# sjpollard/video-how-do-your-tokens-merge

Measured on AMD Instinct MI355X. Metric: clips/sec at r=16, VideoMAE-B 16x224x224 (forward with ToMe merge; merge indices bit-exact against the fp32-arithmetic oracle, which the reference's fp32 fixtures pin), higher is better.
Workload: dtype bf16; 1 GPU; VideoMAE-B random-init, synthetic 16x224x224 clips, r=16, bf16 (BASELINE.json configs[1]); r=16, parallelism=dp1: independent replicas, one RCCL all-reduce of [top1, top5, clips], step_launch=eager

## Files before the change

### include/tome_hip.h

```cpp
#ifndef TOME_HIP_H
#define TOME_HIP_H

#include <stddef.h>
#include <stdint.h>

#ifdef __cplusplus
extern "C" {
#endif

typedef void *tome_stream_t;

enum tome_dtype { TOME_F32 = 0, TOME_BF16 = 1, TOME_F16 = 2 };

enum tome_mode { TOME_SUM = 0, TOME_MEAN = 1, TOME_AMAX = 2, TOME_PROD = 3, TOME_AMIN = 4 };

enum tome_status {
    TOME_OK = 0,
    TOME_EINVAL = 1,
    TOME_EWORKSPACE = 2,
    TOME_ELAUNCH = 3
};

#define TOME_ABI_VERSION 11

// ... 59 lines not shown
                 void *x_out, void *y_out, const void *x_out_bias, tome_stream_t stream);

int tome_drop_regrouped_ln(const void *x, int dtype, int64_t B, int64_t F, int64_t P, int64_t C, int64_t r,
                           int has_cls, const int64_t *und_idx, const void *ln_weight, const void *ln_bias, float eps,
                           const void *addend, int addend_grouped, const void *cls_addend, void *x_out, void *y_out,
                           const void *x_out_bias, tome_stream_t stream);

int tome_prop_attention(const void *q, const void *k, const void *v, int dtype, int64_t B, int64_t H, int64_t N,
                        int64_t Nk, int64_t D, const int64_t *q_strides, const int64_t *k_strides,
                        const int64_t *v_strides, const float *log_size, int64_t log_size_stride, int bias_skip,
                        float scale, void *out, const int64_t *out_strides, tome_stream_t stream);

int tome_prop_attention_segments(const void *q, const void *k, const void *v, int dtype, int64_t B, int64_t H,
                                 int64_t N, int64_t Nk, int64_t D, const int64_t *q_strides,
                                 const int64_t *k_strides, const int64_t *v_strides, const float *log_size,
                                 int64_t log_size_stride, float scale, void *out, const int64_t *out_strides,
                                 int64_t nseg, const int64_t *seg_strides, tome_stream_t stream);

int tome_trajectory_mix(const void *q2, const void *k2, const void *val, int dtype, int64_t B, int64_t S, int64_t F,
                        int64_t H, int64_t D, int64_t k_row_stride, int64_t v_row_stride, float scale, void *out,
                        int64_t out_batch_stride, float *tattn, tome_stream_t stream);

int tome_short_attention(const void *q, const void *k, const void *v, int dtype, int64_t B, int64_t H, int64_t N,
                         int64_t D, const int64_t *q_strides, const int64_t *k_strides, const int64_t *v_strides,
                         float scale, void *out, tome_stream_t stream);

int tome_add_layernorm(const void *x, const void *addend, int dtype, int64_t rows, int64_t C,
                       const void *ln_weight, const void *ln_bias, float eps, void *x_out, void *y_out,
                       tome_stream_t stream);

int tome_add_layernorm_skip_first(const void *x, const void *addend, int dtype, int64_t groups, int64_t group_rows,
                                  int64_t C, const void *ln_weight, const void *ln_bias, float eps, void *x_out,
                                  void *y_out, tome_stream_t stream);

int tome_add_layernorm_regrouped(const void *x, const void *addend, int dtype, int64_t B, int64_t F, int64_t P,
                                 int64_t C, const void *ln_weight, const void *ln_bias, float eps, void *x_out,
                                 void *y_out, tome_stream_t stream);

int tome_merge(const void *x, int dtype, int64_t n, int64_t T, int64_t C, int64_t r,
               const int64_t *src_idx, const int64_t *dst_idx, const int64_t *unm_idx,
               int distill_token, int mode, const uint8_t *edge_keep, void *out,
               tome_stream_t stream);

int tome_drop(const void *x, int dtype, int64_t n, int64_t T, int64_t C, int64_t r,
              const int64_t *und_idx, int distill_token, void *out, tome_stream_t stream);

int tome_unmerge(const void *x, int dtype, int64_t n, int64_t T, int64_t C, int64_t r,
                 const int64_t *src_idx, const int64_t *dst_idx, const int64_t *unm_idx, void *out,
                 tome_stream_t stream);

int tome_merge_backward(const void *grad_out, int x_dtype, const void *out_div, const void *in_mul, int size_dtype,
                        int64_t n, int64_t T, int64_t C, int64_t r, const int32_t *row_map, int distill_token,
                        int drop, void *grad_in, tome_stream_t stream);
int tome_merge_backward_regrouped(const void *grad_out, int x_dtype, const void *out_div, const void *in_mul,
                                  int size_dtype, int64_t B, int64_t F, int64_t P, int64_t C, int64_t r, int has_cls,
                                  const int32_t *row_map, int drop, void *grad_in, tome_stream_t stream);

size_t tome_layernorm_backward_workspace_bytes(int64_t rows, int64_t C);
int tome_layernorm_backward(const void *gy, const void *xs, const void *gx_in, int dtype, int64_t groups,
                            int64_t group_rows, int skip_first, int64_t C, const void *weight, float eps, void *gx,
                            void *dweight, void *dbias, void *workspace, tome_stream_t stream);

size_t tome_layernorm_backward_regrouped_workspace_bytes(int64_t B, int64_t F, int64_t P, int64_t C);
int tome_layernorm_backward_regrouped(const void *gy, const void *xs, const void *gx_in, int dtype, int64_t B, int64_t F,
                                      int64_t P, int64_t C, const void *weight, float eps, void *gx, void *dweight,
                                      void *dbias, void *workspace, tome_stream_t stream);
// ... 112 lines not shown
```

### video-how-do-your-tokens-merge_amd/csrc/tome_kernels.hip

```cpp
#include <hip/hip_runtime.h>
#include <stdarg.h>
#include <stdint.h>
#include <stdio.h>
#include <stdlib.h>
#include <string.h>

#include <type_traits>

#include "../../include/tome_hip.h"
#include "tome_common.h"
#include "tome_match.h"
#include "tome_match_filter.h"
#include "tome_ln_rows.h"
#include "tome_merge_slab.h"
#include "tome_merge.h"
#include "tome_merge_ln_amp.h"
#include "tome_ln_fwd.h"
#include "tome_merge_bwd.h"
#include "tome_ln_bwd.h"
#include "tome_merge_ln_bwd.h"
#include "tome_merge_ln_bwd_amp.h"
#include "tome_gelu.h"
#include "tome_gelu_bwd.h"
#include "tome_token_mean.h"
// ... 606 lines not shown
}

extern "C" int tome_merge_wavg_regrouped_ln(const void *x, int x_dtype, const void *size, int size_dtype, int64_t B,
                                            int64_t F, int64_t P, int64_t C, int64_t r, int has_cls,
                                            const int64_t *src_idx, const int64_t *dst_idx,
                                            const int64_t *unm_idx, const uint8_t *edge_keep, const void *ln_weight,
                                            const void *ln_bias, float eps, const void *addend,
                                            int addend_grouped, const void *cls_addend, void *x_out,
                                            void *y_out, void *size_out, void *log_size_out,
                                            const void *x_out_bias, tome_stream_t stream) {
    if (x_out_bias && !aligned16(x_out_bias))
        return fail(TOME_EINVAL, "tome_merge_wavg_regrouped_ln: x_out_bias not 16-byte aligned");
    if (!y_out || !ln_weight || !ln_bias) return fail(TOME_EINVAL, "tome_merge_wavg_regrouped_ln: null buffer");
    if (x_dtype == TOME_F32) return fail(TOME_EINVAL, "tome_merge_wavg_regrouped_ln: 16-bit tokens only");
    if ((addend && !aligned16(addend)) || (cls_addend && !aligned16(cls_addend)))
        return fail(TOME_EINVAL, "tome_merge_wavg_regrouped_ln: addend alignment");
    if (addend_grouped && !addend) return fail(TOME_EINVAL, "tome_merge_wavg_regrouped_ln: addend_grouped without addend");
    LnArgs ln{ln_weight, ln_bias, y_out, eps, addend, 0, TokLayout{0, 0, 0, 0, 1}, nullptr, x_out_bias};
    if (addend_grouped) {
        const int64_t cls = has_cls ? 1 : 0;
        ln.a_own = 1;
        ln.la = TokLayout{cls * C, (cls + P) * C, 0, C, 1};
        ln.cls_addend = cls_addend;
    }
    return merge_wavg_regrouped_impl("tome_merge_wavg_regrouped_ln", x, x_dtype, size, size_dtype, B, F, P, C, r,
                                     has_cls, src_idx, dst_idx, unm_idx, edge_keep, x_out, size_out, log_size_out, &ln, stream);
}

static inline int ln_rows_per_wave(int64_t cpr, int nit) {
    const int64_t R = (nit * WAVE) / cpr;
    return R > FAST_MAXR ? FAST_MAXR : (int)R;
}

template <typename TS, typename TA, typename TY, typename TP>
static int launch_add_ln_rows(const char *who, const void *x, const void *addend, int64_t rows, int64_t C,
                              const void *ln_weight, const void *ln_bias, float eps, int64_t y_group, void *x_out,
                              void *y_out, tome_stream_t stream) {
    const int64_t cpr = C / 8;
    const int R = ln_rows_per_wave(cpr, 3);
    const int64_t waves = (rows + R - 1) / R;
    if ((waves + 3) / 4 > 0x7fffffffLL) return fail(TOME_EINVAL, "%s: too many rows", who);
    hipLaunchKernelGGL((k_add_ln_rows<TS, TA, TY, TP, 3>), dim3((unsigned)((waves + 3) / 4)), dim3(256), 0,
                       (hipStream_t)stream, (const TS *)x, (const TA *)addend, rows, (int)C, R, (int)cpr,
                       (const TP *)ln_weight, (const TP *)ln_bias, eps, (int)y_group, (TS *)x_out, (TY *)y_out);
    return check_launch("k_add_ln_rows");
}

static int add_layernorm_impl(const void *x, const void *addend, int dtype, int64_t rows, int64_t C,
                              const void *ln_weight, const void *ln_bias, float eps, void *x_out, void *y_out,
                              int64_t y_group, tome_stream_t stream) {
    if (!x || !ln_weight || !ln_bias || (addend && !x_out) || !y_out || rows <= 0 || C <= 0)
        return fail(TOME_EINVAL, "tome_add_layernorm: bad shape/pointer");
    if (int rc = not_16bit("tome_add_layernorm", dtype)) return rc;
    if (C % 8 || C / 8 > 2 * WAVE || !aligned16(x) || !aligned16(addend) || (addend && !aligned16(x_out)) ||
        !aligned16(y_out) || !aligned16(ln_weight) || !aligned16(ln_bias))
        return fail(TOME_EINVAL, "tome_add_layernorm: C %% 8 == 0, C <= 1024 and 16-byte aligned buffers required");
    return dispatch_x<false>(dtype, [&](auto tx) {
        using TX = typename decltype(tx)::type;
        return launch_add_ln_rows<TX, TX, TX, TX>("tome_add_layernorm", x, addend, rows, C, ln_weight, ln_bias, eps,
                                                  y_group, x_out, y_out, stream);
    }, [&] { return not_16bit("tome_add_layernorm", dtype); });
}

extern "C" int tome_add_layernorm(const void *x, const void *addend, int dtype, int64_t rows, int64_t C,
                                  const void *ln_weight, const void *ln_bias, float eps, void *x_out, void *y_out,
                                  tome_stream_t stream) {
    return add_layernorm_impl(x, addend, dtype, rows, C, ln_weight, ln_bias, eps, x_out, y_out, 0, stream);
}

extern "C" int tome_add_layernorm_skip_first(const void *x, const void *addend, int dtype, int64_t groups,
                                             int64_t group_rows, int64_t C, const void *ln_weight,
                                             const void *ln_bias, float eps, void *x_out, void *y_out,
                                             tome_stream_t stream) {
    if (groups <= 0 || group_rows < 2 || group_rows > 0x7fffffffLL)
        return fail(TOME_EINVAL, "tome_add_layernorm_skip_first: groups of at least two rows required");
    return add_layernorm_impl(x, addend, dtype, groups * group_rows, C, ln_weight, ln_bias, eps, x_out, y_out, group_rows,
                              stream);
}

extern "C" int tome_add_layernorm_regrouped(const void *x, const void *addend, int dtype, int64_t B, int64_t F, int64_t P,
                                            int64_t C, const void *ln_weight, const void *ln_bias, float eps,
                                            void *x_out, void *y_out, tome_stream_t stream) {
    if (!x || !addend || !x_out || !y_out || !ln_weight || !ln_bias || B <= 0 || F <= 0 || P <= 0 || C <= 0)
        return fail(TOME_EINVAL, "tome_add_layernorm_regrouped: bad shape/pointer");
    if (int rc = not_16bit("tome_add_layernorm_regrouped", dtype)) return rc;
    const int64_t cpr = C / 8;
    if (C % 8 || cpr > 2 * WAVE || !aligned16(x) || !aligned16(addend) || !aligned16(x_out) || !aligned16(y_out) ||
        !aligned16(ln_weight) || !aligned16(ln_bias))
        return fail(TOME_EINVAL, "tome_add_layernorm_regrouped: C %% 8 == 0, C <= 1024 and 16-byte aligned buffers required");
    const int64_t rows = B * (1 + P * F);
    if (rows > 0x7fffffffLL) return fail(TOME_EINVAL, "tome_add_layernorm_regrouped: too many rows");
    const int R = ln_rows_per_wave(cpr, 3);
    if (R < 1) return fail(TOME_EINVAL, "tome_add_layernorm_regrouped: row too wide");
    const int64_t waves = (rows + R - 1) / R;
    const LnArgs ln{ln_weight, ln_bias, y_out, eps, nullptr, 0, TokLayout{0, 0, 0, 0, 1}, nullptr, nullptr};
    const dim3 grid((unsigned)((waves + 3) / 4));
    hipStream_t st = (hipStream_t)stream;
    return dispatch_x<false>(dtype, [&](auto tx) {
        using TX = typename decltype(tx)::type;
        hipLaunchKernelGGL((k_add_ln_regroup<TX, 3>), grid, dim3(256), 0, st, (const TX *)x, (const TX *)addend, (int)B,
// ... 1353 lines not shown
```

### video-how-do-your-tokens-merge_amd/csrc/tome_ln_fwd.h

```cpp
#pragma once
template <typename TS, typename TA, typename TY, typename TP, int NIT>
__global__ __launch_bounds__(256) void k_add_ln_rows(const TS *__restrict__ x, const TA *__restrict__ a, int64_t rows,
                                                     int C, int R, int cpr, const TP *__restrict__ lw,
                                                     const TP *__restrict__ lb, float eps, int y_group,
                                                     TS *__restrict__ xout, TY *__restrict__ y) {
    const int lane = threadIdx.x & 63;
    const int64_t w = (int64_t)blockIdx.x * (blockDim.x >> 6) + __builtin_amdgcn_readfirstlane(threadIdx.x >> 6);
    const int64_t row0 = w * R;
    if (row0 >= rows) return;
    const int nrow = (int)((rows - row0) < R ? (rows - row0) : R);
    const int total = nrow * cpr;
    const bool add = a != nullptr;
    const TS *xs = x + row0 * C;
    const TA *as = a + row0 * C;
    Slot<TS> raw[NIT] = {};
    Slot<TA> rawa[NIT] = {};
    int rowof[NIT];
#pragma unroll
    for (int it = 0; it < NIT; ++it) {
        const int q = it * WAVE + lane;
        rowof[it] = q < total ? slab_row(cpr, it, lane) : -1;
        if (q < total) {
            raw[it] = ld_slot<TS>(xs, q);
            if (add) rawa[it] = ld_slot<TA>(as, q);
        }
    }
    const LnParams<TP, NIT> prm = ln_params<TP, NIT>(lw, lb, rowof, cpr, lane);
    if (add) {
#pragma unroll
        for (int it = 0; it < NIT; ++it) {
            if (rowof[it] < 0) continue;
            raw[it] = slot_add<TS, TA>(raw[it], rawa[it]);
            st_slot<TS>(xout + row0 * C, it * WAVE + lane, raw[it]);
        }
    }
    ln_rows<TS, TP, TY, NIT>(raw, rowof, nrow, cpr, C, eps, prm, lane,
                             [&](int rr, int cc, const Slot<TY> &yv) __attribute__((always_inline)) {
                                 int64_t yrow = row0 + rr;
                                 if (y_group > 0) {
                                     const int64_t gb = yrow / y_group;
                                     if (yrow - gb * y_group == 0) return;
                                     yrow -= gb + 1;
                                 }
                                 st_slot<TY>(y + yrow * C, cc, yv);
                             });
}

template <typename TX, int NIT>
__global__ __launch_bounds__(256) void k_add_ln_regroup(const TX *__restrict__ x, const TX *__restrict__ a, int B, int F,
                                                        int P, int C, int R, int cpr, LnArgs ln,
                                                        TX *__restrict__ xout) {
    const int lane = threadIdx.x & 63;
    const int64_t w = (int64_t)blockIdx.x * (blockDim.x >> 6) + __builtin_amdgcn_readfirstlane(threadIdx.x >> 6);
    const int N = 1 + P * F;
    const int64_t rows = (int64_t)B * N;
    const int64_t row0 = w * R;
    if (row0 >= rows) return;
// ... 52 lines not shown
```

### video-how-do-your-tokens-merge_amd/tome/_abi.py

```python
from __future__ import annotations

import ctypes
import os
from typing import Optional

import torch

_PKG = os.path.dirname(os.path.dirname(os.path.abspath(__file__)))
LIB_PATH = os.environ.get("TOME_HIP_LIB", os.path.join(_PKG, "lib", "libtome_hip.so"))

i64, i32, vp, sz, f32 = ctypes.c_int64, ctypes.c_int, ctypes.c_void_p, ctypes.c_size_t, ctypes.c_float
SIGNATURES = {
    "tome_abi_version": (i32, [], False),
    "tome_last_error": (ctypes.c_char_p, [], False),
    "tome_effective_r": (i64, [i64, i64, i32, i32], False),
    "tome_match_workspace_bytes": (sz, [i64, i64, i64], False),
    "tome_match": (i32, [vp, i32, i64, i64, i64, i64, i64, i64, i32, i32, vp, vp, vp, vp, vp, vp, sz, vp], False),
    "tome_match_keys": (i32, [vp, i32, i64, i64, i64, i64, i64, i64, i64, i64, i64, i64, i32, i32, vp, vp, vp, vp, vp,
                             vp, sz, vp], False),
    "tome_match_scores": (i32, [vp, i64, i64, i64, i32, i32, vp, vp, vp, vp, vp, vp, sz, vp], False),
    "tome_edge_keep": (i32, [vp, vp, i64, i64, i64, f32, vp, vp], False),
    "tome_merge_wavg": (i32, [vp, i32, vp, i32, i64, i64, i64, i64, vp, vp, vp, i32, vp, vp, vp, vp, vp], False),
    "tome_merge_wavg_ln": (i32, [vp, i32, vp, i32, i64, i64, i64, i64, vp, vp, vp, i32, vp, vp, vp, f32, vp, vp, vp, vp,
                                vp, vp, vp], False),
# ... 34 lines not shown
    "tome_prop_attention_backward": (i32, [vp, vp, vp, vp, vp, i32, i64, i64, i64, i64, i64, vp, vp, vp, vp, vp, vp,
                                          i64, i32, f32, vp, vp, vp, vp, vp, vp, vp, sz, vp], True),
    "tome_gelu_erf_backward_workspace_bytes": (sz, [i64, i64], True),
    "tome_gelu_erf_backward": (i32, [vp, vp, i32, i64, i64, vp, vp, vp, vp, sz, vp], True),
    "tome_short_attention_backward": (i32, [vp, vp, vp, vp, i32, i64, i64, i64, i64, vp, vp, vp, f32, vp, vp, vp, vp,
                                           vp, vp, vp], True),
    "tome_layernorm_backward_regrouped_workspace_bytes": (sz, [i64, i64, i64, i64], True),
    "tome_layernorm_backward_regrouped": (i32, [vp, vp, vp, i32, i64, i64, i64, i64, vp, f32, vp, vp, vp, vp, vp],
                                               True),
    "tome_prop_attention_segments_backward_workspace_bytes": (sz, [i64, i64, i64, i64, i64], True),
    "tome_prop_attention_segments_backward": (i32, [vp, vp, vp, vp, vp, i32, i64, i64, i64, i64, i64, vp, vp, vp, vp, vp,
                                                   vp, i64, f32, i64, vp, vp, vp, vp, vp, vp, vp, vp, vp, sz, vp], True),
    "tome_trajectory_mix_backward": (i32, [vp, vp, vp, vp, i32, i64, i64, i64, i64, i64, i64, i64, i64, f32, vp, vp, vp,
                                          i64, i64, vp], True),
    "tome_gelu_tanh": (i32, [vp, i32, i64, vp, vp], True),
    "tome_gelu_tanh_backward": (i32, [vp, vp, i32, i64, i64, vp, vp, vp, vp, sz, vp], True),
    "tome_add_layernorm_amp": (i32, [vp, i32, vp, i32, i64, i64, i32, i64, vp, vp, f32, vp, vp, i32, vp], True),
    "tome_layernorm_backward_amp_workspace_bytes": (sz, [i64, i64, i32], True),
    "tome_layernorm_backward_amp": (i32, [vp, i32, vp, vp, i32, i64, i64, i32, i64, vp, f32, vp, vp, vp, vp, vp, vp],
                                         True),
    "tome_token_mean": (i32, [vp, i32, i64, i64, i64, i32, vp, vp], True),
    "tome_drop_ln": (i32, [vp, i32, i64, i64, i64, i64, vp, i32, vp, vp, f32, vp, vp, vp, vp, vp], True),
    "tome_drop_regrouped_ln": (i32, [vp, i32, i64, i64, i64, i64, i64, i32, vp, vp, vp, f32, vp, i32, vp, vp, vp, vp, vp],
                               True),
    "tome_merge_ln_backward_workspace_bytes": (sz, [i64, i64, i64], True),
    "tome_merge_ln_backward": (i32, [vp, vp, vp, i32, vp, vp, i32, i64, i64, i64, i64, vp, i32, i32, vp, f32, vp, vp, vp,
                                    vp, vp], True),
    "tome_merge_wavg_ln_amp": (i32, [vp, i32, vp, i32, vp, i32, i64, i64, i64, i64, vp, vp, vp, i32, vp, vp, vp, f32, vp,
                                    vp, i32, vp, vp, vp], True),
    "tome_drop_ln_amp": (i32, [vp, i32, vp, i32, i64, i64, i64, i64, vp, i32, vp, vp, f32, vp, vp, i32, vp], True),
    "tome_merge_ln_backward_amp_workspace_bytes": (sz, [i64, i64, i64, i32], True),
    "tome_merge_ln_backward_amp": (i32, [vp, i32, vp, vp, i32, vp, vp, i32, i64, i64, i64, i64, vp, i32, i32, vp, f32, vp,
                                        vp, vp, vp, vp, vp], True),
}
SYMBOLS = tuple(SIGNATURES)

ABI_VERSION = 11
DTYPES = {torch.float32: 0, torch.bfloat16: 1, torch.float16: 2}
MODES = {"sum": 0, "mean": 1, "amax": 2, "max": 2, "prod": 3, "amin": 4, "min": 4}

_lib = None


class TomeHipError(RuntimeError):
    pass


def lib() -> ctypes.CDLL:
    global _lib
    if _lib is not None:
        return _lib
    _lib = bind(LIB_PATH)
    return _lib


def bind(path: str) -> ctypes.CDLL:
    if not os.path.exists(path):
        raise TomeHipError(
            f"HIP extension not found at {path}: the MI355X merge path has no fallback. "
            "Build it with `python video-how-do-your-tokens-merge_amd/csrc/build.py` (needs hipcc).")
    L = ctypes.CDLL(path)
    for name, (restype, argtypes, later) in SIGNATURES.items():
        if later and not _exports(L, name):
            continue
        fn = getattr(L, name)
        fn.restype, fn.argtypes = restype, argtypes
# ... 331 lines not shown
    log = _log_size_like(s_out, log_size)
    with _on_device(x.device):
        rc = lib().tome_merge_wavg_ln(x.data_ptr(), xcode, _ptr(size), DTYPES[sdtype], n, T, C, plan.r,
                                      plan.src_idx.data_ptr(), plan.dst_idx.data_ptr(), plan.unm_idx.data_ptr(),
                                      int(plan.distill_token), _ptr(plan.edge_keep), weight.data_ptr(), bias.data_ptr(),
                                      float(eps), _ptr(addend), x_out.data_ptr(), y_out.data_ptr(), s_out.data_ptr(),
                                      _ptr(log), _ptr(out_bias), _stream(x.device))
    _check(rc, "tome_merge_wavg_ln")
    return x_out, y_out, s_out


def add_layernorm(x: torch.Tensor, addend: Optional[torch.Tensor], weight: torch.Tensor, bias: torch.Tensor, eps: float,
                  skip_first: bool = False):
    require_device(x, "add_layernorm(x)")
    x = x if x.is_contiguous() else x.contiguous()
    C = x.shape[-1]
    addend = _addend("add_layernorm", addend, x)
    if skip_first and (x.dim() != 3 or x.shape[1] < 2):
        raise TomeHipError("add_layernorm(skip_first): x must be [B, N >= 2, C]")
    x_out = None if addend is None else torch.empty_like(x)
    y_out = (torch.empty((x.shape[0], x.shape[1] - 1, C), dtype=x.dtype, device=x.device) if skip_first
             else torch.empty_like(x))
    with _on_device(x.device):
        if skip_first:
            rc = lib().tome_add_layernorm_skip_first(x.data_ptr(), _ptr(addend), dtype_code(x, "x"), x.shape[0],
                                                     x.shape[1], C, weight.data_ptr(), bias.data_ptr(), float(eps),
                                                     _ptr(x_out), y_out.data_ptr(), _stream(x.device))
        else:
            rc = lib().tome_add_layernorm(x.data_ptr(), _ptr(addend), dtype_code(x, "x"), x.numel() // C, C,
                                          weight.data_ptr(), bias.data_ptr(), float(eps), _ptr(x_out), y_out.data_ptr(),
                                          _stream(x.device))
    _check(rc, "tome_add_layernorm_skip_first" if skip_first and addend is not None else "tome_add_layernorm")
    return (x if addend is None else x_out), y_out


def _f32_params(what: str, C: int, device, *params):
    for p in params:
        if p.numel() != C or p.dtype != torch.float32 or p.device != device:
            raise TomeHipError(f"{what}: the LayerNorm's parameters must hold {C} values of torch.float32 on {device}")
    return [p.detach().contiguous() for p in params]


def _amp_rows(what: str, x: torch.Tensor, skip_first: bool):
    C = x.shape[-1]
    if x.dim() < 2 or C % 8 or C > 1024 or x.numel() == 0:
        raise TomeHipError(f"{what}: tokens must be [..., C] with C % 8 == 0 and C <= 1024, got {tuple(x.shape)}")
    if skip_first:
        if x.dim() != 3 or x.shape[1] < 2:
            raise TomeHipError(f"{what}(skip_first): tokens must be [B, N >= 2, C]")
        return x.shape[0], x.shape[1]
    return x.numel() // C, 1


def add_layernorm_amp(x: torch.Tensor, addend: Optional[torch.Tensor], weight: torch.Tensor, bias: torch.Tensor,
                      eps: float, y_dtype: torch.dtype, skip_first: bool = False):
    require_device(x, "add_layernorm_amp(x)")
    if y_dtype not in _HALF:
        raise TomeHipError(f"add_layernorm_amp: y_dtype must be a 16-bit dtype, got {y_dtype}")
    x = x if x.is_contiguous() else x.contiguous()
    C = x.shape[-1]
    groups, group_rows = _amp_rows("add_layernorm_amp", x, skip_first)
    weight, bias = _f32_params("add_layernorm_amp", C, x.device, weight, bias)
    addend = _addend("add_layernorm_amp", addend, x, same_dtype=False)
    L = lib()
    entry = require_symbol(L, "tome_add_layernorm_amp")
    x_out = None if addend is None else torch.empty_like(x)
# ... 1088 lines not shown
```

### video-how-do-your-tokens-merge_amd/tome/patch/_common.py

```python
from __future__ import annotations

import os
import threading
from typing import Callable, Dict, Tuple

import torch

from .. import _abi, _attn, _ln, _mlp, _overlap
from .. import merge as tm
from .._mlp import _plain_mlp, _stock_module
from ..merge import (bipartite_soft_matching, bipartite_soft_matching_drop, bipartite_soft_matching_hybrid, do_nothing,
                     drop_regrouped, merge_source, merge_wavg, merge_wavg_regrouped)
from ..utils import parse_r

_SUBCLASSES: Dict[Tuple[type, str], type] = {}
_FUSE_LN = os.environ.get("TOME_FUSE_LN", "1") != "0"
_FUSE_ADD = os.environ.get("TOME_FUSE_ADD", "1") != "0"
_FUSE_MODES = os.environ.get("TOME_FUSE_MODES", "1") != "0"
_FUSE_NEXT = os.environ.get("TOME_FUSE_NEXT", "1") != "0"
_ATTN_KERNEL = os.environ.get("TOME_ATTN_KERNEL", "1") != "0"
_GELU_KERNEL = os.environ.get("TOME_GELU_KERNEL", "1") != "0"
_FUSE_FC2 = os.environ.get("TOME_FUSE_FC2", "1") != "0"
_POOL_TAIL = os.environ.get("TOME_POOL_TAIL", "1") != "0"
_SKIP_FIRST = os.environ.get("TOME_SKIP_FIRST", "1") != "0"


def swizzle(module: torch.nn.Module, tag: str, methods: dict) -> None:
    base = module.__class__
    if getattr(base, "_tome_tag", None) == tag:
        return
    key = (base, tag)
    sub = _SUBCLASSES.get(key)
    if sub is None:
        sub = type(tag, (base,), dict(methods, _tome_tag=tag))
        _SUBCLASSES[key] = sub
    module.__class__ = sub


def has_tag(module, tag: str) -> bool:
    return getattr(module.__class__, "_tome_tag", None) == tag


def new_tome_info(trace_source, prop_attn, mode, head_aggregation, threshold, verbose, class_token) -> dict:
    return {
        "r": 0,
        "size": None,
        "source": None,
        "trace_source": trace_source,
        "prop_attn": prop_attn,
        "verbose": verbose,
        "class_token": class_token,
        "distill_token": False,
        "mode": mode,
        "head_aggregation": head_aggregation,
        "threshold": threshold,
    }

# ... 46 lines not shown


def _note_forward_issued(device) -> None:
    sid, cur = _current_stream(device)
    _in_flight[device.index] = (sid, _record_event(cur))


class one_forward_at_a_time:

    def __init__(self, device):
        self.device = device
        self.on = device is not None and _guarded(device)

    def __enter__(self):
        if self.on:
            self.lock = _issue_lock(self.device)
            self.lock.acquire()
            try:
                _guard_one_forward_in_flight(self.device)
            except BaseException:
                self.lock.release()
                raise
        return self

    def __exit__(self, *exc):
        if self.on:
            try:
                _note_forward_issued(self.device)
            finally:
                self.lock.release()
        return False


def wrap_model_forward(model_wrapper: torch.nn.Module, blocks_of: Callable, pool_tail: Callable = None) -> None:
    base = model_wrapper.__class__
    if getattr(base, "_tome_tag", None) == "ToMeVisionTransformer":
        return

    def forward(self, *args, **kwdargs):
        param = next(self.parameters(), None)
        with one_forward_at_a_time(None if param is None else param.device):
            self._tome_info["r"] = parse_r(len(blocks_of(self)), self.r)
            self._tome_info["size"] = None
            self._tome_info["source"] = None
            self._tome_info.pop("_prenorm", None)
            self._tome_info.pop("_folded", None)
            armed = pool_tail(self) if (pool_tail is not None and _POOL_TAIL) else None
            if armed is not None:
                self._tome_info["_pool_tail"] = armed
            try:
                return super(sub, self).forward(*args, **kwdargs)
            finally:
                self._tome_info.pop("_pool_tail", None)
                if param is not None:
                    _overlap.join(param.device)

    sub = type("ToMeVisionTransformer", (base,), {"forward": forward, "_tome_tag": "ToMeVisionTransformer"})
    model_wrapper.__class__ = sub


keys_ready = _overlap.keys_ready
match_beside = _overlap.match_beside


def attention_qkv(qkv, size, scale: float, dropout_p: float = 0.0, bias_skip: bool = False):
    return attention(qkv[0], qkv[1], qkv[2], size, scale, dropout_p, bias_skip, qkv)


def attention(q, k, v, size, scale: float, dropout_p: float = 0.0, bias_skip: bool = False, qkv=None):
    out = _attn.attention(q, k, v, size, scale, dropout_p, bias_skip, qkv) if _ATTN_KERNEL else None
    if out is not None:
        return out
    B, H, N, hd = q.shape
    bias = None
    if size is not None:
        log = _abi.log_of_size(size)[:, None, None, :, 0].to(q.dtype)
        if bias_skip:
            bias = torch.zeros(B, 1, N, N, dtype=q.dtype, device=q.device)
            bias[:, :, 1:, 1:] = log
        else:
            bias = log
    out = torch.nn.functional.scaled_dot_product_attention(q, k, v, attn_mask=bias, dropout_p=dropout_p, scale=scale)
    return out.transpose(1, 2).reshape(B, N, H * hd)

# ... 32 lines not shown
def _unhooked(*modules) -> bool:
    return not any(m._forward_hooks or m._forward_pre_hooks for m in modules)


def pool_tail_modules_ok(vit, block) -> bool:
    from torch.nn.modules import module as _m
    if _m._global_forward_hooks or _m._global_forward_pre_hooks:
        return False
    norm, fc_norm = getattr(vit, "norm", None), getattr(vit, "fc_norm", None)
    if not (type(norm) is torch.nn.Identity and isinstance(fc_norm, torch.nn.LayerNorm) and not vit.training
            and not block.training and has_tag(block, "ToMeBlock") and getattr(block, "gamma_2", 0) is None
            and type(getattr(block, "drop_path", None)) is torch.nn.Identity
            and _unhooked(vit, norm, block, block.drop_path) and _plain_mlp(block.mlp)):
        return False
    fc1, fc2, norm2 = block.mlp.fc1, block.mlp.fc2, getattr(block, "norm2", None)
    dtype = fc2.weight.dtype
    return (fc2.bias is not None and dtype in _abi._HALF and fc1.weight.dtype == dtype
            and isinstance(norm2, torch.nn.LayerNorm) and norm2.elementwise_affine and norm2.weight.dtype == dtype
            and fc1.in_features % 8 == 0 and fc1.out_features % 8 == 0 and fc2.out_features == fc1.in_features)


def pool_tail_armed(block, x, info) -> bool:
    if info.get("_pool_tail") is not block:
        return False
    info.pop("_pool_tail")
    return (x.is_cuda and x.dim() == 3 and x.dtype == block.mlp.fc2.weight.dtype and not torch.is_grad_enabled()
            and not torch.is_autocast_enabled("cuda"))


def pooled_tail(mlp, x, y):
    h = mlp.fc1(y)
    abar = _abi.token_mean(h if h.is_contiguous() else h.contiguous(), gelu=True)
    xbar = _abi.token_mean(x if x.is_contiguous() else x.contiguous())
    fc2 = mlp.fc2
    pooled = torch.addmm(xbar + fc2.bias.float(), abar, fc2.weight.float().t())
    return pooled.to(x.dtype)[:, None, :]


def pick_reduction(mode: str, merge_fn, drop_fn, hybrid_fn):
    if mode in ("merge", "random_merge"):
        return merge_fn
    if mode in ("drop", "random_drop"):
        return drop_fn
    if mode in ("hybrid",):
        return hybrid_fn
    raise ValueError(f"unknown ToMe mode {mode!r}")


def matching(kind: str, metric, r: int, info):
    if kind == "drop":
        found = bipartite_soft_matching_drop(metric, r, info["class_token"], info["distill_token"], info["mode"])
    elif kind == "hybrid":
        found = bipartite_soft_matching_hybrid(metric, r, info["class_token"], info["distill_token"], info["mode"],
                                               info["threshold"])
    else:
        found = bipartite_soft_matching(metric, r, info["class_token"], info["distill_token"], info["mode"])
    if isinstance(found, tuple):
        found = found[0]
    return None if found is do_nothing else found


def reduce_merge(metric, x, info, r):
    return _apply_merge(matching("merge", metric, r, info) or do_nothing, x, info)


def _apply_merge(merge, x, info):
    if info["trace_source"]:
        info["source"] = merge_source(merge, x, info["source"])
    before = x.size(1)
# ... 305 lines not shown
```

### video-how-do-your-tokens-merge_amd/tome/patch/videomae.py

```python
from __future__ import annotations

import copy
import sys

import torch
import torch.nn.functional as F

from . import _common as C
from ..merge import HeadMeanKeys


def _block_forward(self, x):
    info = self._tome_info
    attn_size = info["size"] if info["prop_attn"] else None
    attn, metric = self.attn(C.first_norm(self, x, info, self.norm1), attn_size, info["head_aggregation"])
    if self.gamma_1 is not None:
        attn = self.gamma_1 * attn
    pooled = C.pool_tail_armed(self, x, info)
    fold = (C.foldable(self.mlp.fc2, not self.training)
            if (not pooled and self.gamma_2 is None and C._plain_mlp(self.mlp)) else None)
    x, y = C.merge_then_norm(metric, x, info, self.norm2, self.reduction_function, videomae_merge,
                             residual=self.drop_path(attn), fold=fold, drop_fn=videomae_drop, hybrid_fn=videomae_hybrid)
    if pooled:
        return C.pooled_tail(self.mlp, x, y)
    return C.mlp_residual(self, self.mlp, x, y, info, scale=self.gamma_2, drop_path=self.drop_path)


def _duplicate_block_forward(self, x):
    info = self._tome_info
    attn_size = info["size"] if info["prop_attn"] else None
    _, metric = self.attn(self.norm1(x), attn_size, info["head_aggregation"])
    return self.reduction_function(metric, x, info)


def _attention_forward(self, x, size: torch.Tensor = None, head_aggregation: str = "mean"):
    B, N, _ = x.shape
    bias = None
    if self.q_bias is not None:
        bias = torch.cat((self.q_bias, torch.zeros_like(self.v_bias, requires_grad=False), self.v_bias))
    qkv = F.linear(x, self.qkv.weight, bias).reshape(B, N, 3, self.num_heads, -1).permute(2, 0, 3, 1, 4)
    q, k, v = qkv[0], qkv[1], qkv[2]
    drop_p = self.attn_drop.p if self.training else 0.0
    info = getattr(self, "_tome_info", None)
    ready = C.keys_ready(k, info) if head_aggregation == "mean" else None
    out = C.attention_qkv(qkv, size, self.scale, drop_p)
    if head_aggregation == "mean":
        metric = HeadMeanKeys(k)
        C.match_beside(metric, ready, info)
    elif head_aggregation == "concat":
        metric = k.transpose(1, 2).reshape(B, N, -1)
    else:
        raise ValueError(f"head_aggregation {head_aggregation!r}")
    return self.proj_drop(self.proj(out)), metric


def videomae_merge(metric, x, _tome_info):
    r = _tome_info["r"].pop(0)
    return C.reduce_merge(metric, x, _tome_info, r) if r > 0 else x


def videomae_drop(metric, x, _tome_info):
    r = _tome_info["r"].pop(0)
    return C.reduce_drop(metric, x, _tome_info, r) if r > 0 else x


def videomae_hybrid(metric, x, _tome_info):
    r = _tome_info["r"].pop(0)
    return C.reduce_hybrid(metric, x, _tome_info, r) if r > 0 else x


def pooled_tail_block(wrapper):
    if torch.is_grad_enabled():
        return None
    host = sys.modules.get("hosts.videomae")
    vit = getattr(wrapper, "model", None)
    if (host is None or type(vit) is not host.VisionTransformer or type(wrapper).__bases__ != (host.VideoMAE,)
            or "forward" in vit.__dict__ or "forward_features" in vit.__dict__ or "forward" in wrapper.__dict__
            or len(vit.blocks) == 0):
        return None
    block = vit.blocks[-1]
    if (getattr(block, "_tome_info", None) is not wrapper._tome_info or "forward" in block.__dict__
            or any(b is block for b in vit.blocks[:-1])):
        return None
    return block if C.pool_tail_modules_ok(vit, block) else None


def _is_block(m) -> bool:
    return all(hasattr(m, a) for a in ("attn", "mlp", "norm1", "norm2", "gamma_1"))


def _is_attention(m) -> bool:
    return all(hasattr(m, a) for a in ("qkv", "proj", "num_heads", "q_bias"))


def apply_duplicate_patch(model, layer_to_duplicate, quantity):
    for i in range(layer_to_duplicate, layer_to_duplicate + quantity - 1):
        model.model.blocks.insert(index=i, module=copy.deepcopy(model.model.blocks[i]))
        C.swizzle(model.model.blocks[i], "ToMeDuplicateBlock", {"forward": _duplicate_block_forward})


def apply_patch(model_wrapper, trace_source: bool = False, prop_attn: bool = False, mode: str = "merge",
                head_aggregation: str = "mean", threshold: float = 0.0, verbose: bool = False):
    model = model_wrapper.model
    C.wrap_model_forward(model_wrapper, lambda w: w.model.blocks, pool_tail=pooled_tail_block)
    model_wrapper.r = 0
    model_wrapper._tome_info = C.new_tome_info(trace_source, prop_attn, mode, head_aggregation, threshold, verbose,
                                               class_token=False)
    reduction_function = C.pick_reduction(mode, videomae_merge, videomae_drop, videomae_hybrid)
    for module in model.modules():
        if C.has_tag(module, "ToMeDuplicateBlock"):
            module._tome_info = model_wrapper._tome_info
            module.reduction_function = reduction_function
        elif _is_block(module):
            C.swizzle(module, "ToMeBlock", {"forward": _block_forward})
            module._tome_info = model_wrapper._tome_info
            module.reduction_function = reduction_function
        elif _is_attention(module):
            C.swizzle(module, "ToMeAttention", {"forward": _attention_forward})
            module._tome_info = model_wrapper._tome_info
    C.link_next_norms(model.blocks, "norm1")
```

Baseline: 2640 clips/s.

## Fuse positional-embedding add with first LayerNorm and cache parameter casts

Adds a periodic add+LayerNorm kernel that reads the positional-embedding table by row modulo period, so the pos-embed add and block-0 norm1 run as one launch, with the prenormed output handed to the first block. The model forward is rerouted through a folded front path when hooks, grad and autocast are off. Concatenated qkv biases and fp32 fc2 weight casts are cached per module, keyed on tensor version and pointer. This removes several small elementwise kernels and cast allocations per forward, at the cost of a custom forward path that duplicates the host model's logic and depends on cache invalidation being correct.

```diff
diff --git a/include/tome_hip.h b/include/tome_hip.h
--- a/include/tome_hip.h
+++ b/include/tome_hip.h
@@ -115,6 +115,10 @@
 int tome_add_layernorm_skip_first(const void *x, const void *addend, int dtype, int64_t groups, int64_t group_rows,
                                   int64_t C, const void *ln_weight, const void *ln_bias, float eps, void *x_out,
                                   void *y_out, tome_stream_t stream);
+
+int tome_add_layernorm_periodic(const void *x, const void *table, int dtype, int64_t rows, int64_t period, int64_t C,
+                                const void *ln_weight, const void *ln_bias, float eps, void *x_out, void *y_out,
+                                tome_stream_t stream);
 
 int tome_add_layernorm_regrouped(const void *x, const void *addend, int dtype, int64_t B, int64_t F, int64_t P,
                                  int64_t C, const void *ln_weight, const void *ln_bias, float eps, void *x_out,
diff --git a/video-how-do-your-tokens-merge_amd/csrc/tome_kernels.hip b/video-how-do-your-tokens-merge_amd/csrc/tome_kernels.hip
--- a/video-how-do-your-tokens-merge_amd/csrc/tome_kernels.hip
+++ b/video-how-do-your-tokens-merge_amd/csrc/tome_kernels.hip
@@ -662,17 +662,18 @@
     return R > FAST_MAXR ? FAST_MAXR : (int)R;
 }
 
-template <typename TS, typename TA, typename TY, typename TP>
+template <typename TS, typename TA, typename TY, typename TP, bool PERIODIC = false>
 static int launch_add_ln_rows(const char *who, const void *x, const void *addend, int64_t rows, int64_t C,
                               const void *ln_weight, const void *ln_bias, float eps, int64_t y_group, void *x_out,
-                              void *y_out, tome_stream_t stream) {
+                              void *y_out, tome_stream_t stream, int64_t period = 0) {
     const int64_t cpr = C / 8;
     const int R = ln_rows_per_wave(cpr, 3);
     const int64_t waves = (rows + R - 1) / R;
     if ((waves + 3) / 4 > 0x7fffffffLL) return fail(TOME_EINVAL, "%s: too many rows", who);
-    hipLaunchKernelGGL((k_add_ln_rows<TS, TA, TY, TP, 3>), dim3((unsigned)((waves + 3) / 4)), dim3(256), 0,
+    hipLaunchKernelGGL((k_add_ln_rows<TS, TA, TY, TP, 3, PERIODIC>), dim3((unsigned)((waves + 3) / 4)), dim3(256), 0,
                        (hipStream_t)stream, (const TS *)x, (const TA *)addend, rows, (int)C, R, (int)cpr,
-                       (const TP *)ln_weight, (const TP *)ln_bias, eps, (int)y_group, (TS *)x_out, (TY *)y_out);
+                       (const TP *)ln_weight, (const TP *)ln_bias, eps, (int)y_group, (int)period, (TS *)x_out,
+                       (TY *)y_out);
     return check_launch("k_add_ln_rows");
 }
 
@@ -696,6 +697,27 @@
                                   const void *ln_weight, const void *ln_bias, float eps, void *x_out, void *y_out,
                                   tome_stream_t stream) {
     return add_layernorm_impl(x, addend, dtype, rows, C, ln_weight, ln_bias, eps, x_out, y_out, 0, stream);
+}
+
+extern "C" int tome_add_layernorm_periodic(const void *x, const void *table, int dtype, int64_t rows, int64_t period,
+                                           int64_t C, const void *ln_weight, const void *ln_bias, float eps,
+                                           void *x_out, void *y_out, tome_stream_t stream) {
+    const char *who = "tome_add_layernorm_periodic";
+    if (period == 0)
+        return add_layernorm_impl(x, table, dtype, rows, C, ln_weight, ln_bias, eps, x_out, y_out, 0, stream);
+    if (!x || !table || !ln_weight || !ln_bias || !x_out || !y_out || rows <= 0 || C <= 0)
+        return fail(TOME_EINVAL, "%s: bad shape/pointer (a period needs its table)", who);
+    if (period < 0 || period > 0x7fffffffLL || rows % period)
+        return fail(TOME_EINVAL, "%s: the period %lld must divide the %lld rows", who, (long long)period, (long long)rows);
+    if (int rc = not_16bit(who, dtype)) return rc;
+    if (C % 8 || C / 8 > 2 * WAVE || !aligned16(x) || !aligned16(table) || !aligned16(x_out) || !aligned16(y_out) ||
+        !aligned16(ln_weight) || !aligned16(ln_bias))
+        return fail(TOME_EINVAL, "%s: C %% 8 == 0, C <= 1024 and 16-byte aligned buffers required", who);
+    return dispatch_x<false>(dtype, [&](auto tx) {
+        using TX = typename decltype(tx)::type;
+        return launch_add_ln_rows<TX, TX, TX, TX, true>(who, x, table, rows, C, ln_weight, ln_bias, eps, 0, x_out, y_out,
+                                                        stream, period);
+    }, [&] { return not_16bit(who, dtype); });
 }
 
 extern "C" int tome_add_layernorm_skip_first(const void *x, const void *addend, int dtype, int64_t groups,
diff --git a/video-how-do-your-tokens-merge_amd/csrc/tome_ln_fwd.h b/video-how-do-your-tokens-merge_amd/csrc/tome_ln_fwd.h
--- a/video-how-do-your-tokens-merge_amd/csrc/tome_ln_fwd.h
+++ b/video-how-do-your-tokens-merge_amd/csrc/tome_ln_fwd.h
@@ -1,8 +1,8 @@
 #pragma once
-template <typename TS, typename TA, typename TY, typename TP, int NIT>
+template <typename TS, typename TA, typename TY, typename TP, int NIT, bool PERIODIC = false>
 __global__ __launch_bounds__(256) void k_add_ln_rows(const TS *__restrict__ x, const TA *__restrict__ a, int64_t rows,
                                                      int C, int R, int cpr, const TP *__restrict__ lw,
-                                                     const TP *__restrict__ lb, float eps, int y_group,
+                                                     const TP *__restrict__ lb, float eps, int y_group, int period,
                                                      TS *__restrict__ xout, TY *__restrict__ y) {
     const int lane = threadIdx.x & 63;
     const int64_t w = (int64_t)blockIdx.x * (blockDim.x >> 6) + __builtin_amdgcn_readfirstlane(threadIdx.x >> 6);
@@ -13,6 +13,13 @@
     const bool add = a != nullptr;
     const TS *xs = x + row0 * C;
     const TA *as = a + row0 * C;
+    int64_t arow0 = 0, arow1 = 0, arow2 = 0, arow3 = 0;
+    if constexpr (PERIODIC) {
+        arow0 = row0 % period;
+        arow1 = (row0 + 1) % period;
+        arow2 = (row0 + 2) % period;
+        arow3 = (row0 + 3) % period;
+    }
     Slot<TS> raw[NIT] = {};
     Slot<TA> rawa[NIT] = {};
     int rowof[NIT];
@@ -22,7 +29,12 @@
         rowof[it] = q < total ? slab_row(cpr, it, lane) : -1;
         if (q < total) {
             raw[it] = ld_slot<TS>(xs, q);
-            if (add) rawa[it] = ld_slot<TA>(as, q);
+            if constexpr (PERIODIC) {
+                const int rr = rowof[it];
+                rawa[it] = ld_param_slot<TA>(a + SEL4(rr, arow0, arow1, arow2, arow3) * C, slab_col(q, rr, cpr));
+            } else {
+                if (add) rawa[it] = ld_slot<TA>(as, q);
+            }
         }
     }
     const LnParams<TP, NIT> prm = ln_params<TP, NIT>(lw, lb, rowof, cpr, lane);
diff --git a/video-how-do-your-tokens-merge_amd/tome/_abi.py b/video-how-do-your-tokens-merge_amd/tome/_abi.py
--- a/video-how-do-your-tokens-merge_amd/tome/_abi.py
+++ b/video-how-do-your-tokens-merge_amd/tome/_abi.py
@@ -90,6 +90,7 @@
     "tome_merge_ln_backward_amp_workspace_bytes": (sz, [i64, i64, i64, i32], True),
     "tome_merge_ln_backward_amp": (i32, [vp, i32, vp, vp, i32, vp, vp, i32, i64, i64, i64, i64, vp, i32, i32, vp, f32, vp,
                                         vp, vp, vp, vp, vp], True),
+    "tome_add_layernorm_periodic": (i32, [vp, vp, i32, i64, i64, i64, vp, vp, f32, vp, vp, vp], True),
 }
 SYMBOLS = tuple(SIGNATURES)
 
@@ -487,6 +488,22 @@
                                           _stream(x.device))
     _check(rc, "tome_add_layernorm_skip_first" if skip_first and addend is not None else "tome_add_layernorm")
     return (x if addend is None else x_out), y_out
+
+
+def add_layernorm_periodic(x: torch.Tensor, table: torch.Tensor, weight: torch.Tensor, bias: torch.Tensor, eps: float):
+    require_device(x, "add_layernorm_periodic(x)")
+    x = x if x.is_contiguous() else x.contiguous()
+    C = x.shape[-1]
+    if (table.dim() != 2 or table.shape[1] != C or table.dtype != x.dtype or table.device != x.device
+            or not table.is_contiguous() or table.shape[0] == 0):
+        raise TomeHipError(f"add_layernorm_periodic: table must be a contiguous [P, {C}] tensor of x's dtype and device")
+    entry = require_symbol(lib(), "tome_add_layernorm_periodic")
+    x_out, y_out = torch.empty_like(x), torch.empty_like(x)
+    with _on_device(x.device):
+        rc = entry(x.data_ptr(), table.data_ptr(), dtype_code(x, "x"), x.numel() // C, table.shape[0], C,
+                   weight.data_ptr(), bias.data_ptr(), float(eps), x_out.data_ptr(), y_out.data_ptr(), _stream(x.device))
+    _check(rc, "tome_add_layernorm_periodic")
+    return x_out, y_out
 
 
 def _f32_params(what: str, C: int, device, *params):
diff --git a/video-how-do-your-tokens-merge_amd/tome/patch/_common.py b/video-how-do-your-tokens-merge_amd/tome/patch/_common.py
--- a/video-how-do-your-tokens-merge_amd/tome/patch/_common.py
+++ b/video-how-do-your-tokens-merge_amd/tome/patch/_common.py
@@ -22,7 +22,26 @@
 _GELU_KERNEL = os.environ.get("TOME_GELU_KERNEL", "1") != "0"
 _FUSE_FC2 = os.environ.get("TOME_FUSE_FC2", "1") != "0"
 _POOL_TAIL = os.environ.get("TOME_POOL_TAIL", "1") != "0"
+_FUSE_FRONT = os.environ.get("TOME_FUSE_FRONT", "1") != "0"
+_CACHE_QKV_BIAS = os.environ.get("TOME_CACHE_QKV_BIAS", "1") != "0"
+_CACHE_CASTS = os.environ.get("TOME_CACHE_CASTS", "1") != "0"
 _SKIP_FIRST = os.environ.get("TOME_SKIP_FIRST", "1") != "0"
+
+
+def kept_key(sources, extra=()):
+    return tuple((t._version, t.data_ptr(), t.dtype, t.device) for t in sources) + tuple(extra) + (
+        torch.is_inference_mode_enabled(),)
+
+
+def kept(module, slot: str, sources, build: Callable, extra=()):
+    key = kept_key(sources, extra)
+    held = module.__dict__.get(slot)
+    if held is not None and held[0] == key and len(held[1]) == len(sources) and all(a is b for a, b in zip(held[1], sources)):
+        return held[2]
+    value = build()
+    if not (value.is_cuda and torch.cuda.is_current_stream_capturing()):
+        object.__setattr__(module, slot, (key, tuple(sources), value))
+    return value
 
 
 def swizzle(module: torch.nn.Module, tag: str, methods: dict) -> None:
@@ -135,7 +154,8 @@
         return False
 
 
-def wrap_model_forward(model_wrapper: torch.nn.Module, blocks_of: Callable, pool_tail: Callable = None) -> None:
+def wrap_model_forward(model_wrapper: torch.nn.Module, blocks_of: Callable, pool_tail: Callable = None,
+                       front: Callable = None) -> None:
     base = model_wrapper.__class__
     if getattr(base, "_tome_tag", None) == "ToMeVisionTransformer":
         return
@@ -151,8 +171,9 @@
             armed = pool_tail(self) if (pool_tail is not None and _POOL_TAIL) else None
             if armed is not None:
                 self._tome_info["_pool_tail"] = armed
+            folded = front(self, args, kwdargs) if (front is not None and _FUSE_FRONT) else None
             try:
-                return super(sub, self).forward(*args, **kwdargs)
+                return super(sub, self).forward(*args, **kwdargs) if folded is None else folded()
             finally:
                 self._tome_info.pop("_pool_tail", None)
                 if param is not None:
@@ -251,9 +272,17 @@
     h = mlp.fc1(y)
     abar = _abi.token_mean(h if h.is_contiguous() else h.contiguous(), gelu=True)
     xbar = _abi.token_mean(x if x.is_contiguous() else x.contiguous())
-    fc2 = mlp.fc2
-    pooled = torch.addmm(xbar + fc2.bias.float(), abar, fc2.weight.float().t())
+    w2, b2 = _f32_of(mlp.fc2)
+    pooled = torch.addmm(xbar + b2, abar, w2.t())
     return pooled.to(x.dtype)[:, None, :]
+
+
+def _f32_of(linear):
+    w, b = linear.weight, linear.bias
+    if not _CACHE_CASTS or (torch.is_grad_enabled() and (w.requires_grad or b.requires_grad)):
+        return w.float(), b.float()
+    return (kept(linear, "_tome_weight_f32", (w,), lambda: w.detach().float()),
+            kept(linear, "_tome_bias_f32", (b,), lambda: b.detach().float()))
 
 
 def pick_reduction(mode: str, merge_fn, drop_fn, hybrid_fn):
diff --git a/video-how-do-your-tokens-merge_amd/tome/patch/videomae.py b/video-how-do-your-tokens-merge_amd/tome/patch/videomae.py
--- a/video-how-do-your-tokens-merge_amd/tome/patch/videomae.py
+++ b/video-how-do-your-tokens-merge_amd/tome/patch/videomae.py
@@ -7,6 +7,7 @@
 import torch.nn.functional as F
 
 from . import _common as C
+from .. import _abi, _ln
 from ..merge import HeadMeanKeys
 
 
@@ -35,9 +36,7 @@
 
 def _attention_forward(self, x, size: torch.Tensor = None, head_aggregation: str = "mean"):
     B, N, _ = x.shape
-    bias = None
-    if self.q_bias is not None:
-        bias = torch.cat((self.q_bias, torch.zeros_like(self.v_bias, requires_grad=False), self.v_bias))
+    bias = qkv_bias(self)
     qkv = F.linear(x, self.qkv.weight, bias).reshape(B, N, 3, self.num_heads, -1).permute(2, 0, 3, 1, 4)
     q, k, v = qkv[0], qkv[1], qkv[2]
     drop_p = self.attn_drop.p if self.training else 0.0
@@ -69,20 +68,87 @@
     return C.reduce_hybrid(metric, x, _tome_info, r) if r > 0 else x
 
 
-def pooled_tail_block(wrapper):
-    if torch.is_grad_enabled():
-        return None
+def _host_vit(wrapper):
     host = sys.modules.get("hosts.videomae")
     vit = getattr(wrapper, "model", None)
     if (host is None or type(vit) is not host.VisionTransformer or type(wrapper).__bases__ != (host.VideoMAE,)
             or "forward" in vit.__dict__ or "forward_features" in vit.__dict__ or "forward" in wrapper.__dict__
             or len(vit.blocks) == 0):
         return None
+    return vit
+
+
+def pooled_tail_block(wrapper):
+    vit = None if torch.is_grad_enabled() else _host_vit(wrapper)
+    if vit is None:
+        return None
     block = vit.blocks[-1]
     if (getattr(block, "_tome_info", None) is not wrapper._tome_info or "forward" in block.__dict__
             or any(b is block for b in vit.blocks[:-1])):
         return None
     return block if C.pool_tail_modules_ok(vit, block) else None
+
+
+def qkv_bias(attn):
+    q, v = attn.q_bias, attn.v_bias
+    if q is None:
+        return None
+    if not C._CACHE_QKV_BIAS or (torch.is_grad_enabled() and (q.requires_grad or v.requires_grad)):
+        return torch.cat((q, torch.zeros_like(v, requires_grad=False), v))
+    return C.kept(attn, "_tome_qkv_bias", (q, v),
+                  lambda: torch.cat((q.detach(), torch.zeros_like(v, requires_grad=False), v.detach())))
+
+
+def pos_table(vit, pos, dtype):
+    return C.kept(vit, "_tome_pos_table", (pos,), lambda: pos.detach().to(dtype)[0].contiguous(), (dtype,))
+
+
+def front_fold_modules_ok(wrapper) -> bool:
+    if torch.is_grad_enabled() or torch.is_autocast_enabled("cuda"):
+        return False
+    from torch.nn.modules import module as _m
+    if _m._global_forward_hooks or _m._global_forward_pre_hooks:
+        return False
+    vit = _host_vit(wrapper)
+    if vit is None or wrapper.training or vit.training:
+        return False
+    block = vit.blocks[0]
+    norm1 = getattr(block, "norm1", None)
+    if (getattr(block, "_tome_info", None) is not wrapper._tome_info or "forward" in block.__dict__ or block.training
+            or not C.has_tag(block, "ToMeBlock") or not isinstance(norm1, torch.nn.LayerNorm)
+            or not C._unhooked(vit, block, norm1)):
+        return False
+    pos = vit.__dict__["_buffers"].get("pos_embed")
+    return (type(pos) is torch.Tensor and pos.dim() == 3 and pos.shape[0] == 1 and pos.is_floating_point()
+            and not pos.requires_grad)
+
+
+def _front_tokens_ok(x, pos, norm1) -> bool:
+    return (x.dim() == 3 and x.is_cuda and x.dtype in (torch.bfloat16, torch.float16) and pos.device == x.device
+            and tuple(pos.shape) == (1, x.shape[1], x.shape[2]) and pos.dtype in (torch.float32, x.dtype)
+            and _ln.route(x, norm1) == "direct")
+
+
+def front_fold(wrapper, args, kwargs):
+    if len(args) != 1 or kwargs or not front_fold_modules_ok(wrapper):
+        return None
+    return lambda: _folded_forward(wrapper, args[0])
+
+
+def _folded_forward(wrapper, x):
+    vit, info = wrapper.model, wrapper._tome_info
+    x = vit.patch_embed(x[0])
+    pos, norm1 = vit.pos_embed, vit.blocks[0].norm1
+    if _front_tokens_ok(x, pos, norm1):
+        x, y = _abi.add_layernorm_periodic(x, pos_table(vit, pos, x.dtype), norm1.weight, norm1.bias, norm1.eps)
+        info["_prenorm"] = (x, y, norm1, False)
+    else:
+        x = x + pos.to(x.dtype)
+    for blk in vit.blocks:
+        x = blk(x)
+    x = vit.norm(x)
+    x = vit.fc_norm(x.mean(1)) if vit.fc_norm is not None else x[:, 0]
+    return vit.head(x)
 
 
 def _is_block(m) -> bool:
@@ -102,7 +168,7 @@
 def apply_patch(model_wrapper, trace_source: bool = False, prop_attn: bool = False, mode: str = "merge",
                 head_aggregation: str = "mean", threshold: float = 0.0, verbose: bool = False):
     model = model_wrapper.model
-    C.wrap_model_forward(model_wrapper, lambda w: w.model.blocks, pool_tail=pooled_tail_block)
+    C.wrap_model_forward(model_wrapper, lambda w: w.model.blocks, pool_tail=pooled_tail_block, front=front_fold)
     model_wrapper.r = 0
     model_wrapper._tome_info = C.new_tome_info(trace_source, prop_attn, mode, head_aggregation, threshold, verbose,
                                                class_token=False)
```

Result: no change. 2646 clips/s, median of 6 (+0.2%).
